# nnnagle/vq-vae

Measured on AMD Instinct MI355X. Metric: tiles/sec, higher is better.
Workload: dtype bf16

## Files before the change

include/frl_hip.h:

```cpp
#ifndef FRL_HIP_H
#define FRL_HIP_H

#include <stddef.h>
#include <stdint.h>

#ifdef __cplusplus
extern "C" {
#endif

typedef void* frl_stream_t;

enum { FRL_F32 = 0, FRL_BF16 = 1, FRL_F16 = 2  };
enum { FRL_ACT_NONE = 0, FRL_ACT_RELU = 1, FRL_ACT_SIGMOID = 2 };

int frl_version(void);
const char* frl_last_error(void);
int frl_device_arch(char* buf, int n);
int frl_kernel_timing_enable(int on);
int frl_kernel_timing_report(char* buf, int n);

size_t frl_pack_cache_table_bytes(void);
int frl_pack_cache_create(void* arena, size_t bytes);
int frl_pack_cache_destroy(int handle);
int frl_pack_cache_activate(int handle);
// ... 56 lines not shown
                     const float* b2, const float* stats, float* dw1, float* dg1, float* db1, float* dw2, float* dg2, float* db2,
                     int B, int HW, void* ws, size_t ws_bytes, frl_stream_t stream);

int frl_sobel_fwd(const void* x, void* g, int B, int H, int W, int C, int dtype, frl_stream_t stream);
int frl_sobel_bwd(const void* dg, void* dx, int B, int H, int W, int C, int dtype, frl_stream_t stream);
int frl_sobel_bwd_add(const void* dg, void* dx, const void* dx_add, int B, int H, int W, int C, int dtype, frl_stream_t stream);
int frl_edge_smooth_stencil_fwd(const void* x, const void* a_logit, const void* b_logit, void* smoothed, void* residual,
                                void* a_soft, void* b_soft, int B, int H, int W, int C, int R, int coarse_dilation,
                                int dtype, frl_stream_t stream);
int frl_edge_smooth_stencil_bwd(const void* d_smoothed, const void* x, const void* a_soft, const void* b_soft, void* dx,
                                void* da_logit, void* db_logit, const void* dx_add , int B, int H,
                                int W, int C, int R, int coarse_dilation, int dtype, frl_stream_t stream);
int frl_smooth_heads_supported(int C, int hidden, int rank, int dtype);
size_t frl_smooth_heads_workspace_bytes(int64_t npix);
int frl_smooth_heads_fwd(const void* x, const void* feat, const float* wa, const float* ba, const float* wb, const float* bb,
                         void* smoothed, void* residual, int B, int H, int W, int coarse_dilation, void* ws, size_t ws_bytes,
                         frl_stream_t stream);
size_t frl_smooth_heads_bwd_scratch_bytes(int64_t npix);
int frl_smooth_heads_force_gather(int on);
int frl_smooth_heads_bwd(const void* d_smoothed, const void* x, const void* feat, const float* wa, const float* ba, const float* wb,
                         const float* bb, const void* dx_add, void* dx, void* dfeat, float* dwa, float* dba, float* dwb, float* dbb,
                         void* scratch, size_t scratch_bytes, int B, int H, int W, int coarse_dilation, void* ws, size_t ws_bytes,
                         frl_stream_t stream);
int frl_smooth_heads_bwd_masked(const void* d_smoothed, const void* x, const void* feat, const float* wa, const float* ba, const float* wb,
                                const float* bb, const void* dx_add, void* dx, void* dfeat, float* dwa, float* dba, float* dwb, float* dbb,
                                void* scratch, size_t scratch_bytes, int B, int H, int W, int dil, int dfeat_relu, void* ws,
                                size_t ws_bytes, frl_stream_t stream);
int frl_film_fused_supported(int cond_dim, int hidden, int target_dim, int dtype);
size_t frl_film_fused_workspace_bytes(void);
int frl_film_fused_fwd(const void* z_type, const void* h, const float* w1g, const float* b1g, const float* w2g, const float* b2g,
                       const float* w1b, const float* b1b, const float* w2b, const float* b2b, void* z, void* gamma, void* beta, int B,
                       int T, int HW, void* ws, size_t ws_bytes, frl_stream_t stream);
int frl_film_fused_bwd(const void* z_type, const void* h, const void* dz, const float* w1g, const float* b1g, const float* w2g,
                       const float* b2g, const float* w1b, const float* b1b, const float* w2b, const float* b2b, void* dh, float* dw1g,
                       float* db1g, float* dw2g, float* db2g, float* dw1b, float* db1b, float* dw2b, float* db2b, int B, int T, int HW,
                       void* ws, size_t ws_bytes, frl_stream_t stream);
int frl_gate_blend_fwd(const void* smoothed, const void* residual, const void* gate_raw, float min_gate, void* out,
                       void* gate_out, int64_t n, int dtype, frl_stream_t stream);
int frl_gate_blend_bwd(const void* dout, const void* dgate_ext, const void* residual, const void* gate_raw, float min_gate,
                       void* d_residual, void* d_gate_raw, int64_t n, int dtype, frl_stream_t stream);
int frl_gate_blend_bwd_masked(const void* dout, const void* dgate_ext, const void* residual, const void* gate_raw, float min_gate,
                              void* d_residual, void* d_gate_raw, int64_t n, int dtype, int sigmoid_mask, frl_stream_t stream);

int frl_tcn_block_fwd(const void* x, const float* conv_w, const float* conv_b, const float* gn_w, const float* gn_b,
                      const float* gate_w, const float* gate_b, const float* proj_w, const float* proj_b, void* y,
                      int64_t npix, int HW, int T, int Cin, int Cout, int dilation, int G, float eps, int dtype, void* ws,
                      size_t ws_bytes, frl_stream_t stream);
size_t frl_tcn_block_bwd_workspace_bytes(int64_t npix, int Cout);
int frl_tcn_block_bwd(const void* x, const void* dy, const float* conv_w, const float* conv_b, const float* gn_w,
                      const float* gn_b, const float* gate_w, const float* gate_b, const float* proj_w,
                      const float* proj_b, void* dconv, void* dgpre, void* normed, void* dres, float* dgamma, float* dbeta,
                      int64_t npix, int HW, int T, int Cin, int Cout, int dilation, int G, float eps, int dtype, void* ws,
                      size_t ws_bytes, frl_stream_t stream);
int frl_tcn_block_bwd_data(const void* dconv, const void* dres, const float* conv_w, const float* proj_w, void* dx,
                           int64_t npix, int HW, int T, int Cin, int Cout, int dilation, int dtype, void* ws, size_t ws_bytes,
                           frl_stream_t stream);

int frl_tcn_block_bwd_fused_supported(int T, int Cin, int Cout, int G, int has_proj, int dtype);
size_t frl_tcn_block_bwd_fused_workspace_bytes(int64_t npix);
int frl_tcn_block_bwd_fused(const void* x, const void* dy, const float* conv_w, const float* conv_b, const float* gn_w,
                            const float* gn_b, const float* gate_w, const float* gate_b, void* dx, float* d_conv_w,
                            float* d_conv_b, float* d_gn_w, float* d_gn_b, float* d_gate_w, float* d_gate_b, int64_t npix,
                            int HW, int T, int dilation, int G, float eps, void* ws, size_t ws_bytes, frl_stream_t stream);

int frl_defer_begin(void);
int frl_defer_pending(void);
int frl_defer_destinations(void** out, int max);
int frl_defer_flush(frl_stream_t stream);
int frl_defer_abort(void);

int frl_tcn_hot_supported(int T, int Cin, int Cout, int G, int dilation, int has_proj, int dtype);
size_t frl_tcn_hot_fwd_workspace_bytes(void);
size_t frl_tcn_hot_bwd_workspace_bytes(int64_t npix);
int frl_tcn_hot_fwd(const void* x, const void* drop_mask, const float* conv_w, const float* conv_b, const float* gn_w, const float* gn_b,
                    const float* gate_w, const float* gate_b, void* y, int64_t npix, int HW, int dilation, float eps, void* ws,
                    size_t ws_bytes, frl_stream_t stream);
int frl_tcn_hot_bwd_nodx_supported(int64_t npix, int HW);
int frl_tcn_hot_bwd(const void* x, const void* drop_mask, const void* dy, const float* conv_w, const float* conv_b, const float* gn_w,
                    const float* gn_b, const float* gate_w, const float* gate_b, void* dx, float* d_conv_w, float* d_conv_b,
                    float* d_gn_w, float* d_gn_b, float* d_gate_w, float* d_gate_b, int64_t npix, int HW, int dilation,
                    float eps, void* ws, size_t ws_bytes, frl_stream_t stream);
size_t frl_tcn_chain_fwd_workspace_bytes(void);
int frl_tcn_chain_static_tiles(int on);
int frl_tcn_chain_fwd(const void* x, const float* const* conv_w, const float* const* conv_b, const float* const* gn_w,
                      const float* const* gn_b, const float* const* gate_w, const float* const* gate_b, const float* head_w,
                      const float* head_b, void* y1, void* y2, void* y3, void* h, int64_t npix, int HW, int Ch, float eps, void* ws,
                      size_t ws_bytes, frl_stream_t stream);
int frl_tcn_hot_bwd_head_supported(int64_t npix, int HW, int Ch);
size_t frl_tcn_hot_bwd_head_workspace_bytes(int64_t npix);
int frl_tcn_hot_bwd_head(const void* x, const void* dh, const float* head_w, int Ch, const float* conv_w, const float* conv_b,
                         const float* gn_w, const float* gn_b, const float* gate_w, const float* gate_b, void* dx, float* d_conv_w,
                         float* d_conv_b, float* d_gn_w, float* d_gn_b, float* d_gate_w, float* d_gate_b, int64_t npix, int HW,
                         int dilation, float eps, void* ws, size_t ws_bytes, frl_stream_t stream);
int frl_tcn_hot_force_generic_tiles(int on);
int frl_tcn_hot_bwd_variant(int v);
int frl_tcn_hot_bwd4_share(int variant, int share);

size_t frl_adamw_workspace_bytes(void);
int frl_adamw_clip_step(const void* desc_host, int ntensors, const void* chunks, const int* chunk_tensor, int nchunks, float max_norm,
                        float lr, double beta1, double beta2, float eps, int step, float* norm_out, const float* ok, int* counters,
                        const float* lr_dev, void* ws, size_t ws_bytes, frl_stream_t stream);
int frl_multi_tensor_scale_copy(const void* desc_host, int ntensors, const void* chunks, const int* chunk_tensor, int nchunks, float scale,
                                frl_stream_t stream);

int frl_film_modulate_fwd(const void* h, const void* gamma, const void* beta, void* out, int64_t B, int T, int64_t HW,
                          int C, int dtype, frl_stream_t stream);
int frl_film_modulate_bwd(const void* dout, const void* h, const void* gamma, void* dh, void* dgamma, void* dbeta,
                          int64_t B, int T, int64_t HW, int C, int dtype, frl_stream_t stream);
int frl_mean_time_fwd(const void* tile, void* out, int64_t B, int T, int64_t HWC, int dtype, frl_stream_t stream);
int frl_add(const void* a, const void* b, float scale_b, void* out, int64_t n, int dtype, frl_stream_t stream);

typedef struct FrlNormRec {
  float sub, div, mul, add, lo, hi;
  int flags;
  int pad;
} FrlNormRec;
int frl_normalize_tiles(const void* raw, int raw_dtype, const uint8_t* valid, const void* table, void* out, int out_dtype,
                        uint8_t* mask_out, int64_t rows, int F, frl_stream_t stream);
int frl_normalize_chunk_tiles(const void* chunk, int raw_dtype, int T, int CY, int CX, int F, const int32_t* desc, int ntiles,
                              int tile, const void* table, void* out, int out_dtype, uint8_t* mask_out, frl_stream_t stream);

int frl_host_parallel_copy(void* dst, const void* src, size_t nbytes, int nthreads);

size_t frl_mse_workspace_bytes(void);
int frl_mse_fwd(const void* pred, const void* target, const uint8_t* mask, int64_t P, int C, float* out, int dtype,
                void* ws, size_t ws_bytes, frl_stream_t stream);
int frl_mse_bwd(const void* pred, const void* target, const uint8_t* mask, const float* gscale, const float* stats,
                int64_t P, int C, void* dpred, int dtype, frl_stream_t stream);

int frl_decoder_mse_fused_supported(int Cz, int hidden, int F, int dtype);
size_t frl_decoder_mse_workspace_bytes(int64_t P, int Cz);
int frl_decoder_mse_fwd(const void* z, const float* w1, const float* b1, const float* w2, const float* b2, const void* target,
                        const uint8_t* mask, void* xhat, float* out, int64_t P, int Cz, void* ws, size_t ws_bytes,
                        frl_stream_t stream);
int frl_decoder_mse_bwd(const void* z, const float* w1, const float* b1, const float* w2, const float* b2, const void* target,
                        const uint8_t* mask, const float* gscale, const float* stats, void* dz, float* dw1, float* db1,
                        float* dw2, float* db2, int64_t P, int Cz, void* ws, size_t ws_bytes, frl_stream_t stream);
int frl_decoder_mse_bwd_subgroups(int on);

size_t frl_vq_workspace_bytes(int64_t N, int K, int d);
int frl_vq_assign_fwd(const void* z, const float* E, int64_t N, int K, int d, int32_t* idx_out, void* zq_out,
                      float* stats_out, int32_t* counts_out, int dtype, void* ws, size_t ws_bytes, frl_stream_t stream);
size_t frl_vq_prepared_bytes(int K, int d);
int frl_vq_stream_tiles(int nt);
int frl_vq_prepare(const float* E, int64_t N, int K, int d, int dtype, void* prep, size_t prep_bytes, frl_stream_t stream);
int frl_vq_assign_fwd_prepared(const void* z, const float* E, void* prep , int64_t N, int K, int d,
                               int32_t* idx_out, void* zq_out, float* stats_out, int32_t* counts_out, int dtype, void* ws,
                               size_t ws_bytes, frl_stream_t stream);
int frl_vq_bwd(const void* g_out, const void* z, const void* zq , const float* E, const int32_t* idx, const int32_t* counts,
               const float* gscale, float beta, int64_t N, int K, int d, void* g_z_out, float* g_E_out, float* sums_out,
               int dtype, void* ws, size_t ws_bytes, frl_stream_t stream);
int frl_vq_ema_update(const float* sums, const int32_t* counts, int K, int d, float decay, float eps, float* ema_count,
                      float* ema_sum, float* E, const float* ok, frl_stream_t stream);
int frl_vq_revive_dead_codes(float* E, const int64_t* window_counts, int64_t min_count, const void* z, int64_t N, int K, int d,
                             uint64_t seed, float* m, float* v, int32_t* revived, int dtype, frl_stream_t stream);

int frl_gather_locations_fwd(const void* feat, int64_t sC, int64_t sH, int64_t sW, int C, int H, int W, const int64_t* coords, int64_t N,
                             void* out, int dtype, frl_stream_t stream);
int frl_segment_sum_rows(const float* vals, const int64_t* order, const int64_t* keys_sorted, int64_t M, int D, float* out, int64_t out_stride,
                         int accumulate, frl_stream_t stream);
int frl_infonce_fwd(const float* emb, int D, const int64_t* pairs, const float* weights, const unsigned char* is_pos, int64_t T,
                    const int64_t* seg, int64_t nseg, float temperature, int similarity, float* sims, float* logits, float* loss_a, float* coef,
                    float* loss, frl_stream_t stream);
int frl_infonce_pair_grads(const float* emb, int D, const int64_t* pairs, const float* sims, const float* coef, const float* gscale, int64_t T,
                           int64_t nseg, float temperature, int similarity, float* ga, float* gb, frl_stream_t stream);

// ... 12 lines not shown
```

vq-vae_amd/csrc/tcn_hot.hip:

```cpp
#include "tcn_hot_common.hpp"

#ifdef TH_STAMPS
__device__ unsigned long long* th_dbg;
#endif
#define TH_PITCH 72

struct Tile2 { frag8 f[2]; };

__device__ __forceinline__ float th_elem(const Tile2& t, int j) { return (float)t.f[j >> 3][j & 7]; }

__device__ __forceinline__ Tile2 th_pack(const float (&v)[16]) {
  Tile2 o;
#pragma unroll
  for (int j = 0; j < 16; ++j) o.f[j >> 3][j & 7] = (bf16)v[j];
  return o;
}

template <int DIL>
__device__ __forceinline__ void th_conv(f32x4 (&acc)[TH_T][4], const Tile2 (&x)[TH_T], const frag8* __restrict__ wl, int lane) {
#pragma unroll
  for (int k = 0; k < 3; ++k)
#pragma unroll
    for (int m = 0; m < 4; ++m)
#pragma unroll
// ... 196 lines not shown
template <bool KEEP>
__global__ __launch_bounds__(512, 2) void tcn_chain_fwd_kernel(const bf16* __restrict__ X, ThChainArgs a, int64_t npix, int HW, int Ch, float eps, int dyn) {
  extern __shared__ __attribute__((aligned(16))) char smem[];
  frag8* wl = reinterpret_cast<frag8*>(smem);
  frag8* wlh = wl + 3 * THC_IMG;
  float* tab = reinterpret_cast<float*>(wlh + 2 * 64);
  const int tid = threadIdx.x, lane = tid & 63, wave = tid >> 6;
  const int px = lane & 15, kc = lane >> 4;
#pragma unroll
  for (int b = 0; b < 3; ++b) copy_frags_lds<bf16>(wl + b * THC_IMG, a.pk[b], THC_IMG, tid, 512);
  copy_frags_lds<bf16>(wlh, a.pkh, 2 * 64, tid, 512);
  for (int i = tid; i < 3 * 256 + 16; i += 512) {
    float v;
    if (i < 768) {
      const int b = i >> 8, w = (i >> 6) & 3, c = i & 63;
      v = w == 0 ? a.bc[b][c] : w == 1 ? a.gw[b][c] : w == 2 ? a.gb[b][c] : -1.44269504088896f * a.bg[b][c];
    } else {
      v = (i - 768) < Ch ? a.bh[i - 768] : 0.f;
    }
    tab[i] = v;
  }
  int* tctr = reinterpret_cast<int*>(tab + 3 * 256 + 16);
  if (tid == 0) *tctr = 8;
  __syncthreads();
  const int64_t ntile = (npix + 15) >> 4;
  const int64_t tstep = (int64_t)gridDim.x * 8;
  auto tile_of = [&](int i) -> int64_t { return (int64_t)blockIdx.x * 8 + (i & 7) + (int64_t)(i >> 3) * tstep; };
  auto rows = [&](int64_t tile, bool& valid) -> int64_t {
    int64_t pidx = tile * 16 + px;
    valid = pidx < npix;
    if (!valid) pidx = npix - 1;
    const int64_t b = pidx / HW, hw = pidx % HW;
    return (b * TH_T * HW + hw) * 64 + 16 * kc;
  };
  Tile2 x[TH_T];
  {
    bool v;
    const int64_t t0 = tile_of(wave);
    const int64_t r0 = rows(t0 < ntile ? t0 : 0, v);
#pragma unroll
    for (int t = 0; t < TH_T; ++t) x[t] = th_load(X + r0 + (int64_t)t * HW * 64);
  }
  int icur = wave;
  for (int64_t tile = tile_of(wave); tile < ntile;) {
    bool valid, vn;
    int inext = icur + 8;
    if (dyn && lane == 0) inext = __hip_atomic_fetch_add(tctr, 1, __ATOMIC_RELAXED, __HIP_MEMORY_SCOPE_WORKGROUP);
    const int64_t r0 = rows(tile, valid);
    int lw = lane, z0 = 0;
    asm volatile("" : "+v"(lw), "+s"(z0));
    const float* tb_ = tab + z0;
    th_block_regs<1>(x, wl, wl + 24 * 64, tb_, lw, kc, eps);
    if (KEEP && valid) {
#pragma unroll
      for (int t = 0; t < TH_T; ++t) th_store(a.y[0] + r0 + (int64_t)t * HW * 64, x[t]);
    }
    __builtin_amdgcn_sched_barrier(0);
    th_block_regs<2>(x, wl + THC_IMG, wl + THC_IMG + 24 * 64, tb_ + 256, lw, kc, eps);
    if (KEEP && valid) {
#pragma unroll
      for (int t = 0; t < TH_T; ++t) th_store(a.y[1] + r0 + (int64_t)t * HW * 64, x[t]);
    }
    __builtin_amdgcn_sched_barrier(0);
    th_block_regs<4>(x, wl + 2 * THC_IMG, wl + 2 * THC_IMG + 24 * 64, tb_ + 512, lw, kc, eps);
    __builtin_amdgcn_sched_barrier(0);
    const f32x4 hb4 = *reinterpret_cast<const f32x4*>(tb_ + 768 + 4 * kc);
    const int64_t hrow = (r0 - 16 * kc) / 64 * Ch + 4 * kc;
#pragma unroll
    for (int t = 0; t < TH_T; ++t) {
      if (KEEP && valid) th_store(a.y[2] + r0 + (int64_t)t * HW * 64, x[t]);
      f32x4 ha = mfma16(wlh[lw], x[t].f[0], hb4);
      ha = mfma16(wlh[64 + lw], x[t].f[1], ha);
      if (valid && 4 * kc < Ch)
        *reinterpret_cast<bf16x4*>(a.h + hrow + (int64_t)t * HW * Ch) = bf16x4{(bf16)ha[0], (bf16)ha[1], (bf16)ha[2], (bf16)ha[3]};
    }
    {
      icur = __builtin_amdgcn_readfirstlane(inext);
      const int64_t tnext = tile_of(icur);
      const int64_t rn = rows(tnext < ntile ? tnext : tile, vn);
#pragma unroll
      for (int t = 0; t < TH_T; ++t) x[t] = th_load(X + rn + (int64_t)t * HW * 64);
      tile = tnext;
    }
  }
}

__device__ __forceinline__ frag8 th_tr(const bf16* tile, int pix0, int ch0, int r16) {
  const bf16* a0 = tile + (pix0 + (r16 >> 2)) * TH_PITCH + ch0 + 4 * (r16 & 3);
  bf16x4 lo = __builtin_amdgcn_ds_read_tr16_b64_v4bf16((bf16x4 __attribute__((address_space(3)))*)(a0));
  bf16x4 hi = __builtin_amdgcn_ds_read_tr16_b64_v4bf16((bf16x4 __attribute__((address_space(3)))*)(a0 + 4 * TH_PITCH));
  return frag8{lo[0], lo[1], lo[2], lo[3], hi[0], hi[1], hi[2], hi[3]};
}
__device__ __forceinline__ void th_put(bf16* tile, int prow, int kc, const Tile2& t) {
  frag8* p = reinterpret_cast<frag8*>(tile + prow * TH_PITCH + 16 * kc);
  p[0] = t.f[0];
  p[1] = t.f[1];
}

#define TH_TILE (64 * TH_PITCH)

__device__ __forceinline__ Tile2 th_get(const bf16* tile, int prow, int kc) {
  const frag8* p = reinterpret_cast<const frag8*>(tile + prow * TH_PITCH + 16 * kc);
  Tile2 t;
  t.f[0] = p[0];
  t.f[1] = p[1];
  return t;
}

template <int DIL, bool MASK>
__global__ __launch_bounds__(512, 2) void tcn_hot_bwd2_kernel(const bf16* __restrict__ X, const bf16* __restrict__ M, const bf16* __restrict__ DY,
                                                              const frag8* __restrict__ Wpk, const float* __restrict__ bc,
                                                              const float* __restrict__ gn_w, const float* __restrict__ gn_b,
                                                              const float* __restrict__ bg, bf16* DX, float* __restrict__ slab,
                                                              int64_t npix, int HW, float eps) {
  extern __shared__ __attribute__((aligned(16))) char smem[];
  frag8* wl_conv = reinterpret_cast<frag8*>(smem);
  frag8* wl_gate = wl_conv + 24 * 64;
  frag8* wl_gateT = wl_gate + 8 * 64;
  frag8* wl_convT = wl_gateT + 8 * 64;
  float* tab = reinterpret_cast<float*>(wl_convT + 24 * 64);
  float* gacc_lds = tab + 4 * 64;
  bf16* bufA = reinterpret_cast<bf16*>(gacc_lds + 4 * 2 * 64);
  bf16* bufB = bufA + TH_T * TH_TILE;
  const int tid = threadIdx.x, lane = tid & 63, wave = tid >> 6;
  const int q = wave & 3, h = wave >> 2;
  const int px = lane & 15, kc = lane >> 4, r16 = px;
  const int prow = q * 16 + px;
  const int co = 16 * kc + 8 * h;
#ifdef TH_STAMPS
  __shared__ unsigned long long th_ts[8][12];
  if (tid < 96) (&th_ts[0][0])[tid] = 0ull;
  unsigned long long t_prev = 0;
#define TH_ST2(i) do { const unsigned long long t_now = __builtin_amdgcn_s_memtime(); if (lane == 0) th_ts[wave][i] += t_now - t_prev; t_prev = t_now; } while (0)
#else
#define TH_ST2(i) do { } while (0)
#endif

  copy_frags_lds<bf16>(wl_conv, Wpk, 64 * 64, tid, 512);
  if (tid < 64) {
    tab[tid] = bc[tid];
    tab[64 + tid] = gn_w[tid];
    tab[128 + tid] = gn_b[tid];
    tab[192 + tid] = -1.44269504088896f * bg[tid];
  }
  __syncthreads();
  float gw[8], gb[8];
#pragma unroll
  for (int e = 0; e < 8; ++e) { gw[e] = tab[64 + co + e]; gb[e] = tab[128 + co + e]; }
  const float* tnbg = tab + 192 + co;
  const f32x4* tcb = reinterpret_cast<const f32x4*>(tab + co);
  const frag8* wc_own = wl_conv + (2 * h) * 2 * 64 + lane;
  const frag8* wg_own = wl_gate + (2 * h) * 2 * 64 + lane;
  const frag8* wgT_own = wl_gateT + (2 * h) * 2 * 64 + lane;
  const frag8* wcT_own = wl_convT + (2 * h) * 2 * 64 + lane;

  f32x4 accC[3][2], accG[2], accCb = {0.f, 0.f, 0.f, 0.f}, accGb = {0.f, 0.f, 0.f, 0.f};
#pragma unroll
  for (int k = 0; k < 3; ++k)
#pragma unroll
    for (int i = 0; i < 2; ++i) accC[k][i] = f32x4{0.f, 0.f, 0.f, 0.f};
#pragma unroll
  for (int i = 0; i < 2; ++i) accG[i] = f32x4{0.f, 0.f, 0.f, 0.f};
  float dgam[8], dbet[8];
#pragma unroll
  for (int e = 0; e < 8; ++e) { dgam[e] = 0.f; dbet[e] = 0.f; }
  const frag8 ones = (r16 == 0) ? frag8{(bf16)1.f, (bf16)1.f, (bf16)1.f, (bf16)1.f, (bf16)1.f, (bf16)1.f, (bf16)1.f, (bf16)1.f}
// ... 295 lines not shown
  return (unsigned)g;
}
static constexpr size_t TH_FWD_LDS = (size_t)32 * 64 * sizeof(frag8) + 4 * 64 * sizeof(float);
static constexpr size_t TH_BWD_LDS = TH_PACK_BYTES + (size_t)(4 * 64 + 4 * 2 * 64) * sizeof(float) + (size_t)2 * TH_T * TH_TILE * sizeof(bf16);

template <int DIL>
static int th_launch_fwd(const void* x, const void* mask, const frag8* pk, const float* bc, const float* gw, const float* gb, const float* bg,
                         void* y, int64_t npix, int HW, float eps, hipStream_t st) {
  if (mask != nullptr) {
    FRL_LAUNCH((tcn_hot_fwd_kernel<DIL, true>), dim3(th_fwd_grid(npix)), dim3(256), TH_FWD_LDS, st, (const bf16*)x, (const bf16*)mask, pk, bc, gw,
               gb, bg, (bf16*)y, npix, HW, eps);
  } else {
    FRL_LAUNCH((tcn_hot_fwd_kernel<DIL, false>), dim3(th_fwd_grid(npix)), dim3(256), TH_FWD_LDS, st, (const bf16*)x, (const bf16*)nullptr, pk, bc,
               gw, gb, bg, (bf16*)y, npix, HW, eps);
  }
  return 0;
}
template <int DIL>
static int th_launch_bwd(const void* x, const void* mask, const void* dy, const frag8* pk, const float* bc, const float* gw, const float* gb,
                         const float* bg, void* dx, float* slab, unsigned grid, int64_t npix, int HW, float eps, hipStream_t st) {
  if (mask != nullptr) {
    auto kern = tcn_hot_bwd2_kernel<DIL, true>;
    FRL_HIP(hipFuncSetAttribute((const void*)kern, hipFuncAttributeMaxDynamicSharedMemorySize, (int)TH_BWD_LDS));
    FRL_LAUNCH_AS("tcn_hot_bwd2_kernel", kern, dim3(grid), dim3(512), TH_BWD_LDS, st, (const bf16*)x, (const bf16*)mask, (const bf16*)dy, pk, bc, gw, gb, bg, (bf16*)dx,
               slab, npix, HW, eps);
  } else {
    auto kern = tcn_hot_bwd2_kernel<DIL, false>;
    FRL_HIP(hipFuncSetAttribute((const void*)kern, hipFuncAttributeMaxDynamicSharedMemorySize, (int)TH_BWD_LDS));
    FRL_LAUNCH_AS("tcn_hot_bwd2_kernel", kern, dim3(grid), dim3(512), TH_BWD_LDS, st, (const bf16*)x, (const bf16*)nullptr, (const bf16*)dy, pk, bc, gw, gb, bg, (bf16*)dx,
               slab, npix, HW, eps);
  }
  return 0;
}

static int g_th_force_bwd2 = 0;

static const frag8* th_packed(const float* conv_w, const float* gate_w, frag8* ws_pk, hipStream_t stream) {
  FrlPackJob jobs[8];
  const size_t blk = (size_t)4 * 2 * 64 * sizeof(frag8);
  for (int k = 0; k < 3; ++k) jobs[k] = frl_pack_job_pw(conv_w + k, k * blk, FRL_BF16, 2, 64, 64, 4, 64 * 3, 3);
  jobs[3] = frl_pack_job_pw(gate_w, 3 * blk, FRL_BF16, 2, 64, 64, 4, 64, 1);
  jobs[4] = frl_pack_job_pw(gate_w, 4 * blk, FRL_BF16, 2, 64, 64, 4, 1, 64);
  for (int k = 0; k < 3; ++k) jobs[5 + k] = frl_pack_job_pw(conv_w + k, (5 + k) * blk, FRL_BF16, 2, 64, 64, 4, 3, 64 * 3);
  bool hit = false;
  frag8* pk = ws_pk;
  if (void* img = frl_pack_cached(jobs, 8, TH_PACK_BYTES, &hit)) pk = (frag8*)img;
  if (!hit) FRL_LAUNCH(tcn_hot_pack_kernel, dim3(32), dim3(256), 0, stream, pk, conv_w, gate_w);
  return pk;
}

extern "C" {

int frl_tcn_hot_force_generic_tiles(int on) { const int was = g_th_force_bwd2; g_th_force_bwd2 = on; return was; }
static int g_th_bwd_variant = 4;
int frl_tcn_hot_bwd_variant(int v) { const int was = g_th_bwd_variant; if (v == 3 || v == 4) g_th_bwd_variant = v; return was; }

int frl_tcn_hot_supported(int T, int Cin, int Cout, int G, int dilation, int has_proj, int dtype) {
  return dtype == FRL_BF16 && Cin == 64 && Cout == 64 && T == TH_T && G == 8 && !has_proj && (dilation == 1 || dilation == 2 || dilation == 4);
}

int frl_tcn_hot_bwd_nodx_supported(int64_t npix, int HW) { return (th_bwd3_supported(npix, HW) && !g_th_force_bwd2) ? 1 : 0; }

size_t frl_tcn_hot_fwd_workspace_bytes(void) { return TH_PACK_BYTES; }
size_t frl_tcn_hot_bwd_workspace_bytes(int64_t npix) { return (size_t)th_bwd_grid(npix) * TH_SLAB * sizeof(float) + 256 + TH_PACK_BYTES; }

int frl_tcn_hot_fwd(const void* x, const void* drop_mask, const float* conv_w, const float* conv_b, const float* gn_w, const float* gn_b, const float* gate_w,
                    const float* gate_b, void* y, int64_t npix, int HW, int dilation, float eps, void* ws, size_t ws_bytes,
                    hipStream_t stream) {
  if (npix <= 0 || HW <= 0) return frl_fail(-2, "tcn_hot_fwd: empty input");
  if (ws == nullptr || ws_bytes < TH_PACK_BYTES) return frl_fail(-4, "tcn_hot_fwd: workspace too small");
  const frag8* pk = th_packed(conv_w, gate_w, (frag8*)ws, stream);
  int rc = -2;
  if (dilation == 1) rc = th_launch_fwd<1>(x, drop_mask, pk, conv_b, gn_w, gn_b, gate_b, y, npix, HW, eps, stream);
  else if (dilation == 2) rc = th_launch_fwd<2>(x, drop_mask, pk, conv_b, gn_w, gn_b, gate_b, y, npix, HW, eps, stream);
  else if (dilation == 4) rc = th_launch_fwd<4>(x, drop_mask, pk, conv_b, gn_w, gn_b, gate_b, y, npix, HW, eps, stream);
  else return frl_fail(-2, "tcn_hot_fwd: dilation must be 1, 2 or 4");
  if (rc) return rc;
  return frl_check_launch("tcn_hot_fwd");
}

size_t frl_tcn_chain_fwd_workspace_bytes(void) { return 3 * TH_PACK_BYTES + 4096; }
static int g_thc_static = 0;
int frl_tcn_chain_static_tiles(int on) { const int was = g_thc_static; g_thc_static = on ? 1 : 0; return was; }
int frl_tcn_chain_fwd(const void* x, const float* const* conv_w, const float* const* conv_b, const float* const* gn_w, const float* const* gn_b,
                      const float* const* gate_w, const float* const* gate_b, const float* head_w, const float* head_b, void* y1, void* y2, void* y3,
                      void* h, int64_t npix, int HW, int Ch, float eps, void* ws, size_t ws_bytes, hipStream_t stream) {
  if (npix <= 0 || HW <= 0) return frl_fail(-2, "tcn_chain_fwd: empty input");
  if (Ch < 4 || Ch > 16 || (Ch & 3)) return frl_fail(-2, "tcn_chain_fwd: head width must be 4, 8, 12 or 16");
  if (ws == nullptr || ws_bytes < frl_tcn_chain_fwd_workspace_bytes()) return frl_fail(-4, "tcn_chain_fwd: workspace too small");
  const int n_keep = (y1 != nullptr) + (y2 != nullptr) + (y3 != nullptr);
  if (n_keep != 0 && n_keep != 3) return frl_fail(-2, "tcn_chain_fwd: y1, y2, y3 must be all set (training) or all NULL (inference)");
  if (h == nullptr) return frl_fail(-1, "tcn_chain_fwd: h is NULL");
  const bool keep = n_keep == 3;
  ThChainArgs a;
  char* w = (char*)ws;
  for (int b = 0; b < 3; ++b) {
    a.pk[b] = th_packed(conv_w[b], gate_w[b], reinterpret_cast<frag8*>(w + b * TH_PACK_BYTES), stream);
    a.bc[b] = conv_b[b]; a.gw[b] = gn_w[b]; a.gb[b] = gn_b[b]; a.bg[b] = gate_b[b];
  }
  {
    FrlPackJob job = frl_pack_job_pw(head_w, 0, FRL_BF16, 2, Ch, 64, 1, 64, 1);
    bool hit = false;
    frag8* pk = reinterpret_cast<frag8*>(w + 3 * TH_PACK_BYTES);
    if (void* img = frl_pack_cached(&job, 1, (size_t)2 * 64 * sizeof(frag8), &hit)) pk = (frag8*)img;
    if (!hit) FRL_LAUNCH((pack_weights_kernel<bf16, 2>), dim3(1), dim3(128), 0, stream, pk, head_w, Ch, 64, 1, (int64_t)64, (int64_t)1);
    a.pkh = pk;
  }
  a.bh = head_b;
  a.y[0] = (bf16*)y1; a.y[1] = (bf16*)y2; a.y[2] = (bf16*)y3; a.h = (bf16*)h;
  int64_t g = ((npix + 15) / 16 + 7) / 8;
  if (g > 256) g = 256;
  const size_t lds = (size_t)(3 * THC_IMG + 2 * 64) * sizeof(frag8) + (3 * 256 + 16) * sizeof(float) + 16;
  if (keep) {
    FRL_HIP(hipFuncSetAttribute((const void*)tcn_chain_fwd_kernel<true>, hipFuncAttributeMaxDynamicSharedMemorySize, (int)lds));
    FRL_LAUNCH_AS("tcn_chain_fwd_kernel", tcn_chain_fwd_kernel<true>, dim3((unsigned)g), dim3(512), lds, stream, (const bf16*)x, a, npix, HW, Ch, eps, g_thc_static ? 0 : 1);
  } else {
    FRL_HIP(hipFuncSetAttribute((const void*)tcn_chain_fwd_kernel<false>, hipFuncAttributeMaxDynamicSharedMemorySize, (int)lds));
    FRL_LAUNCH_AS("tcn_chain_fwd_kernel<false>", tcn_chain_fwd_kernel<false>, dim3((unsigned)g), dim3(512), lds, stream, (const bf16*)x, a, npix, HW, Ch, eps, g_thc_static ? 0 : 1);
  }
  return frl_check_launch("tcn_chain_fwd");
}

int frl_tcn_hot_bwd(const void* x, const void* drop_mask, const void* dy, const float* conv_w, const float* conv_b, const float* gn_w, const float* gn_b,
                    const float* gate_w, const float* gate_b, void* dx, float* d_conv_w, float* d_conv_b, float* d_gn_w, float* d_gn_b,
                    float* d_gate_w, float* d_gate_b, int64_t npix, int HW, int dilation, float eps, void* ws, size_t ws_bytes,
                    hipStream_t stream) {
  if (npix <= 0 || HW <= 0) return frl_fail(-2, "tcn_hot_bwd: empty input");
  if (npix >= (int64_t)1 << 31) return frl_fail(-2, "tcn_hot_bwd: more than 2^31 pixels per launch");
  if (ws == nullptr || ws_bytes < frl_tcn_hot_bwd_workspace_bytes(npix)) return frl_fail(-4, "tcn_hot_bwd: workspace too small");
  const unsigned grid = th_bwd_grid(npix);
  float* slab = (float*)ws;
  const frag8* pk = th_packed(conv_w, gate_w,
                              reinterpret_cast<frag8*>(reinterpret_cast<char*>(ws) + (((size_t)grid * TH_SLAB * sizeof(float) + 255) / 256) * 256), stream);
  int rc = -2;
  if (dx == nullptr && !(drop_mask == nullptr && th_bwd3_supported(npix, HW) && !g_th_force_bwd2))
    return frl_fail(-2, "tcn_hot_bwd: dx may be NULL (input without gradient) only on the tcn_hot_bwd3 route (no mask, HW % 64 == 0)");
  if (drop_mask == nullptr && th_bwd3_supported(npix, HW) && !g_th_force_bwd2)
    rc = (g_th_bwd_variant == 4 && th_bwd4_supported(npix, HW))
             ? th_bwd4_launch(dilation, x, dy, pk, conv_b, gn_w, gn_b, gate_b, dx, slab, grid, npix, HW, eps, stream)
             : th_bwd3_launch(dilation, x, dy, pk, conv_b, gn_w, gn_b, gate_b, dx, slab, grid, npix, HW, eps, stream);
  else if (dilation == 1) rc = th_launch_bwd<1>(x, drop_mask, dy, pk, conv_b, gn_w, gn_b, gate_b, dx, slab, grid, npix, HW, eps, stream);
  else if (dilation == 2) rc = th_launch_bwd<2>(x, drop_mask, dy, pk, conv_b, gn_w, gn_b, gate_b, dx, slab, grid, npix, HW, eps, stream);
  else if (dilation == 4) rc = th_launch_bwd<4>(x, drop_mask, dy, pk, conv_b, gn_w, gn_b, gate_b, dx, slab, grid, npix, HW, eps, stream);
  else return frl_fail(-2, "tcn_hot_bwd: dilation must be 1, 2 or 4");
  if (rc) return rc;
  launch_slab_reduce_deferrable<float, ThEpi>((const float*)slab, (int)grid, (int64_t)TH_SLAB, ThEpi{d_conv_w, d_gate_w, d_conv_b, d_gate_b, d_gn_w, d_gn_b},
                                   stream);
  return frl_check_launch("tcn_hot_bwd");
}

int frl_tcn_hot_bwd_head_supported(int64_t npix, int HW, int Ch) {
  return (th_bwd4_supported(npix, HW) && !g_th_force_bwd2 && g_th_bwd_variant == 4 && Ch >= 4 && Ch <= 16 && (Ch & 3) == 0) ? 1 : 0;
}
size_t frl_tcn_hot_bwd_head_workspace_bytes(int64_t npix) { return frl_tcn_hot_bwd_workspace_bytes(npix) + 4096; }
int frl_tcn_hot_bwd_head(const void* x, const void* dh, const float* head_w, int Ch, const float* conv_w, const float* conv_b, const float* gn_w,
                         const float* gn_b, const float* gate_w, const float* gate_b, void* dx, float* d_conv_w, float* d_conv_b, float* d_gn_w,
                         float* d_gn_b, float* d_gate_w, float* d_gate_b, int64_t npix, int HW, int dilation, float eps, void* ws, size_t ws_bytes,
                         hipStream_t stream) {
  if (npix <= 0 || HW <= 0) return frl_fail(-2, "tcn_hot_bwd_head: empty input");
  if (!frl_tcn_hot_bwd_head_supported(npix, HW, Ch)) return frl_fail(-2, "tcn_hot_bwd_head: unsupported shape (HW % 64, head width 4..16 in fours)");
  if (ws == nullptr || ws_bytes < frl_tcn_hot_bwd_head_workspace_bytes(npix)) return frl_fail(-4, "tcn_hot_bwd_head: workspace too small");
  const unsigned grid = th_bwd_grid(npix);
  float* slab = (float*)ws;
  char* wpk = reinterpret_cast<char*>(ws) + (((size_t)grid * TH_SLAB * sizeof(float) + 255) / 256) * 256;
  const frag8* pk = th_packed(conv_w, gate_w, reinterpret_cast<frag8*>(wpk), stream);
  const frag8* whp;
  {
    FrlPackJob job = frl_pack_job_pw(head_w, 0, FRL_BF16, 1, 64, Ch, 4, 1, 64);
    bool hit = false;
    frag8* img = reinterpret_cast<frag8*>(wpk + TH_PACK_BYTES);
    if (void* c = frl_pack_cached(&job, 1, (size_t)4 * 64 * sizeof(frag8), &hit)) img = (frag8*)c;
    if (!hit) FRL_LAUNCH((pack_weights_kernel<bf16, 1>), dim3(1), dim3(256), 0, stream, img, head_w, 64, Ch, 4, (int64_t)1, (int64_t)64);
    whp = img;
  }
  const int rc = th_bwd4_launch(dilation, x, dh, pk, conv_b, gn_w, gn_b, gate_b, dx, slab, grid, npix, HW, eps, stream, whp, Ch);
  if (rc) return rc;
  launch_slab_reduce_deferrable<float, ThEpi>((const float*)slab, (int)grid, (int64_t)TH_SLAB, ThEpi{d_conv_w, d_gate_w, d_conv_b, d_gate_b, d_gn_w, d_gn_b},
                                   stream);
  return frl_check_launch("tcn_hot_bwd_head");
}

}
```

vq-vae_amd/frl_hip/_lib.py:

```python
from __future__ import annotations

import ctypes
import os
from ctypes import c_char_p, c_float, c_int, c_int64, c_size_t, c_void_p

_HERE = os.path.dirname(os.path.abspath(__file__))
LIB_PATH = os.path.join(_HERE, "libfrlhip_%s.so" % os.environ["FRL_HIP_LIB_TAG"] if os.environ.get("FRL_HIP_LIB_TAG") else "libfrlhip.so")

F32, BF16, F16 = 0, 1, 2
ACT_NONE, ACT_RELU, ACT_SIGMOID = 0, 1, 2

_lib = None


class FrlHipError(RuntimeError):
    pass


P, I, L, F, S, D = c_void_p, c_int, c_int64, c_float, c_size_t, ctypes.c_double
SIGNATURES = {
    "frl_version": (c_int, []),
    "frl_last_error": (c_char_p, []),
    "frl_device_arch": (c_int, [c_char_p, I]),
    "frl_kernel_timing_enable": (c_int, [I]),
# ... 17 lines not shown
    "frl_vq_workspace_bytes": (S, [L, I, I]),
    "frl_vq_assign_fwd": (c_int, [P, P, L, I, I, P, P, P, P, I, P, S, P]),
    "frl_vq_prepared_bytes": (S, [I, I]),
    "frl_vq_prepare": (c_int, [P, L, I, I, I, P, S, P]),
    "frl_vq_stream_tiles": (c_int, [I]),
    "frl_vq_assign_fwd_prepared": (c_int, [P, P, P, L, I, I, P, P, P, P, I, P, S, P]),
    "frl_vq_bwd": (c_int, [P, P, P, P, P, P, P, F, L, I, I, P, P, P, I, P, S, P]),
    "frl_vq_ema_update": (c_int, [P, P, I, I, F, F, P, P, P, P, P]),
    "frl_vq_revive_dead_codes": (c_int, [P, P, L, P, L, I, I, ctypes.c_uint64, P, P, P, I, P]),
    "frl_groupnorm_fwd": (c_int, [P, P, P, P, P, P, I, I, I, I, F, I, I, P]),
    "frl_groupnorm_bwd_workspace_bytes": (S, [I, I, I]),
    "frl_groupnorm_bwd": (c_int, [P, P, P, P, P, P, P, P, P, I, I, I, I, I, I, P, S, P]),
    "frl_scalar_combine": (c_int, [P, P, I, P, P, P]),
    "frl_scalar_fanout": (c_int, [P, P, I, P, P]),
    "frl_scalar_combine_dev": (c_int, [P, P, P, I, P, P, P]),
    "frl_scalar_combine_aux": (c_int, [P, P, P, P, I, P, P, P, P]),
    "frl_scalar_fanout_dev": (c_int, [P, P, P, I, P, P]),
    "frl_encoder2_supported": (c_int, [I, I, I, I, I, I, I]),
    "frl_encoder2_workspace_bytes": (S, [I]),
    "frl_encoder2_fwd": (c_int, [P, P, P, P, P, P, P, P, P, I, I, F, P, S, P]),
    "frl_encoder2_bwd": (c_int, [P, P, P, P, P, P, P, P, P, P, P, P, P, P, P, I, I, P, S, P]),
    "frl_decoder_mse_fused_supported": (c_int, [I, I, I, I]),
    "frl_decoder_mse_workspace_bytes": (S, [L, I]),
    "frl_decoder_mse_fwd": (c_int, [P, P, P, P, P, P, P, P, P, L, I, P, S, P]),
    "frl_decoder_mse_bwd": (c_int, [P, P, P, P, P, P, P, P, P, P, P, P, P, P, L, I, P, S, P]),
    "frl_mse_workspace_bytes": (S, []),
    "frl_mse_fwd": (c_int, [P, P, P, L, I, P, I, P, S, P]),
    "frl_mse_bwd": (c_int, [P, P, P, P, P, L, I, P, I, P]),
    "frl_film_modulate_fwd": (c_int, [P, P, P, P, L, I, L, I, I, P]),
    "frl_film_modulate_bwd": (c_int, [P, P, P, P, P, P, L, I, L, I, I, P]),
    "frl_film_fused_supported": (c_int, [I, I, I, I]),
    "frl_film_fused_workspace_bytes": (S, []),
    "frl_film_fused_fwd": (c_int, [P] * 13 + [I, I, I, P, S, P]),
    "frl_film_fused_bwd": (c_int, [P] * 20 + [I, I, I, P, S, P]),
    "frl_gate_blend_fwd": (c_int, [P, P, P, F, P, P, L, I, P]),
    "frl_gate_blend_bwd": (c_int, [P, P, P, P, F, P, P, L, I, P]),
    "frl_mean_time_fwd": (c_int, [P, P, L, I, L, I, P]),
    "frl_add": (c_int, [P, P, F, P, L, I, P]),
    "frl_normalize_tiles": (c_int, [P, I, P, P, P, I, P, L, I, P]),
    "frl_gather_locations_fwd": (c_int, [P, L, L, L, I, I, I, P, L, P, I, P]),
    "frl_segment_sum_rows": (c_int, [P, P, P, L, I, P, L, I, P]),
    "frl_infonce_fwd": (c_int, [P, I, P, P, P, L, P, L, F, I, P, P, P, P, P, P]),
    "frl_infonce_pair_grads": (c_int, [P, I, P, P, P, P, L, L, F, I, P, P, P]),
    "frl_mutual_knn_max_points": (S, [I]),
    "frl_mutual_knn": (c_int, [P, I, I, P, P, F, I, P, P, P]),
    "frl_host_parallel_copy": (c_int, [P, P, S, I]),
    "frl_normalize_chunk_tiles": (c_int, [P, I, I, I, I, I, P, I, I, P, P, I, P, P]),
    "frl_conv3x3_fwd": (c_int, [P, P, P, P, I, I, I, I, I, I, I, P, S, P]),
    "frl_conv3x3_fwd_gate_blend": (c_int, [P, P, P, P, P, P, P, I, I, I, I, I, I, P, S, P]),
    "frl_conv3x3_bwd_data": (c_int, [P, P, I, P, P, I, I, I, I, I, I, P, S, P]),
    "frl_conv3x3_bwd_data_fused": (c_int, [P, P, I, P, P, P, P, P, I, I, I, I, I, I, P, S, P]),
    "frl_conv3x3_bwd_weight_workspace_bytes": (S, [I, I, I, I, I]),
    "frl_conv3x3_bwd_weight": (c_int, [P, P, I, P, P, P, I, I, I, I, I, I, P, S, I, P]),
    "frl_sobel_fwd": (c_int, [P, P, I, I, I, I, I, P]),
    "frl_sobel_bwd": (c_int, [P, P, I, I, I, I, I, P]),
    "frl_sobel_bwd_add": (c_int, [P, P, P, I, I, I, I, I, P]),
    "frl_edge_smooth_stencil_fwd": (c_int, [P, P, P, P, P, P, P, I, I, I, I, I, I, I, P]),
    "frl_edge_smooth_stencil_bwd": (c_int, [P, P, P, P, P, P, P, P, I, I, I, I, I, I, I, P]),
    "frl_smooth_heads_supported": (c_int, [I, I, I, I]),
    "frl_smooth_heads_workspace_bytes": (S, [L]),
    "frl_smooth_heads_bwd_scratch_bytes": (S, [L]),
    "frl_smooth_heads_force_gather": (c_int, [I]),
    "frl_smooth_heads_fwd": (c_int, [P, P, P, P, P, P, P, P, I, I, I, I, P, S, P]),
    "frl_smooth_heads_bwd": (c_int, [P, P, P, P, P, P, P, P, P, P, P, P, P, P, P, S, I, I, I, I, P, S, P]),
    "frl_tcn_block_fwd": (c_int, [P, P, P, P, P, P, P, P, P, P, L, I, I, I, I, I, I, F, I, P, S, P]),
    "frl_tcn_block_bwd_data": (c_int, [P, P, P, P, P, L, I, I, I, I, I, I, P, S, P]),
    "frl_tcn_block_bwd_workspace_bytes": (S, [L, I]),
    "frl_tcn_block_bwd_fused_supported": (c_int, [I, I, I, I, I, I]),
    "frl_tcn_block_bwd_fused_workspace_bytes": (S, [L]),
    "frl_tcn_block_bwd_fused": (c_int, [P, P, P, P, P, P, P, P, P, P, P, P, P, P, P, L, I, I, I, I, F, P, S, P]),
    "frl_adamw_workspace_bytes": (S, []),
    "frl_adamw_clip_step": (c_int, [P, I, P, P, I, F, F, D, D, F, I, P, P, P, P, P, S, P]),
    "frl_multi_tensor_scale_copy": (c_int, [P, I, P, P, I, F, P]),
    "frl_tcn_hot_supported": (c_int, [I, I, I, I, I, I, I]),
    "frl_tcn_hot_fwd_workspace_bytes": (S, []),
    "frl_tcn_hot_bwd_workspace_bytes": (S, [L]),
    "frl_tcn_hot_fwd": (c_int, [P, P, P, P, P, P, P, P, P, L, I, I, F, P, S, P]),
    "frl_tcn_hot_bwd": (c_int, [P, P, P, P, P, P, P, P, P, P, P, P, P, P, P, P, L, I, I, F, P, S, P]),
    "frl_tcn_hot_force_generic_tiles": (c_int, [I]),
    "frl_tcn_hot_bwd_variant": (c_int, [I]),
    "frl_decoder_mse_bwd_subgroups": (c_int, [I]),
    "frl_tcn_hot_bwd4_share": (c_int, [I, I]),
    "frl_tcn_chain_static_tiles": (c_int, [I]),
    "frl_conv3x3_bwd_data_outmask": (c_int, [P, P, I, P, P, P, I, I, I, I, I, I, I, P, S, P]),
    "frl_gate_blend_bwd_masked": (c_int, [P, P, P, P, F, P, P, L, I, I, P]),
    "frl_smooth_heads_bwd_masked": (c_int, [P, P, P, P, P, P, P, P, P, P, P, P, P, P, P, S, I, I, I, I, I, P, S, P]),
    "frl_tcn_hot_bwd_head_supported": (c_int, [L, I, I]),
    "frl_tcn_hot_bwd_head_workspace_bytes": (S, [L]),
    "frl_tcn_hot_bwd_head": (c_int, [P, P, P, I, P, P, P, P, P, P, P, P, P, P, P, P, P, L, I, I, F, P, S, P]),
    "frl_defer_begin": (c_int, []),
    "frl_defer_pending": (c_int, []),
    "frl_defer_destinations": (c_int, [P, I]),
    "frl_defer_flush": (c_int, [P]),
    "frl_defer_abort": (c_int, []),
    "frl_tcn_hot_bwd_nodx_supported": (c_int, [L, I]),
    "frl_tcn_chain_fwd_workspace_bytes": (S, []),
    "frl_tcn_chain_fwd": (c_int, [P] * 13 + [L, I, I, F, P, S, P]),
    "frl_tcn_block_bwd": (c_int, [P, P, P, P, P, P, P, P, P, P, P, P, P, P, P, P, L, I, I, I, I, I, I, F, I, P, S, P]),
    "frl_decode_codes": (c_int, [P, P, P, L, I, I, I, P, P]),
}


def load():
    global _lib
    if _lib is not None:
        return _lib
    if not os.path.exists(LIB_PATH):
        raise FrlHipError(
            f"{LIB_PATH} not found: build it with `python vq-vae_amd/build.py` "
            "(hipcc --offload-arch=gfx950). There is no CPU fallback.")
    import torch
    lib = ctypes.CDLL(LIB_PATH)
    for name, (res, args) in SIGNATURES.items():
        fn = getattr(lib, name)
        fn.restype = res
        fn.argtypes = args
    _lib = lib
    return lib


def check(rc: int, what: str = "") -> None:
    if rc != 0:
        msg = load().frl_last_error()
        raise FrlHipError(f"{what} failed with code {rc}: {msg.decode() if msg else ''}")
```

Before: 100,700.

## Add 1024-thread chain forward kernel splitting each tile across wave pairs

Adds a new TCN chain forward kernel in which each 16-pixel tile is processed by two waves. Each wave computes half of the output channels, and the halves are exchanged through LDS using a lightweight per-pair atomic barrier. The grid uses 1024-thread blocks instead of 512, and this variant becomes the default when indices fit in 32 bits. The aim is to raise parallelism and latency hiding by halving per-wave MFMA work and register pressure per tile, at the cost of intra-pair spin synchronisation, extra LDS traffic and a duplicated group-norm reduction.

```diff
diff --git a/include/frl_hip.h b/include/frl_hip.h
--- a/include/frl_hip.h
+++ b/include/frl_hip.h
@@ -162,6 +162,7 @@
                     float eps, void* ws, size_t ws_bytes, frl_stream_t stream);
 size_t frl_tcn_chain_fwd_workspace_bytes(void);
 int frl_tcn_chain_static_tiles(int on);
+int frl_tcn_chain_variant(int v);
 int frl_tcn_chain_fwd(const void* x, const float* const* conv_w, const float* const* conv_b, const float* const* gn_w,
                       const float* const* gn_b, const float* const* gate_w, const float* const* gate_b, const float* head_w,
                       const float* head_b, void* y1, void* y2, void* y3, void* h, int64_t npix, int HW, int Ch, float eps, void* ws,
diff --git a/vq-vae_amd/csrc/tcn_hot.hip b/vq-vae_amd/csrc/tcn_hot.hip
--- a/vq-vae_amd/csrc/tcn_hot.hip
+++ b/vq-vae_amd/csrc/tcn_hot.hip
@@ -302,6 +302,216 @@
       for (int t = 0; t < TH_T; ++t) x[t] = th_load(X + rn + (int64_t)t * HW * 64);
       tile = tnext;
     }
+  }
+}
+
+__device__ __forceinline__ void thc4_sync(unsigned* bar, unsigned& gen, int lane) {
+  gen += 2u;
+  if (lane == 0) __hip_atomic_fetch_add(bar, 1u, __ATOMIC_RELAXED, __HIP_MEMORY_SCOPE_WORKGROUP);
+  for (;;) {
+    const unsigned seen = (unsigned)__builtin_amdgcn_readfirstlane((int)__hip_atomic_load(bar, __ATOMIC_RELAXED, __HIP_MEMORY_SCOPE_WORKGROUP));
+    if ((int)(seen - gen) >= 0) break;
+    __builtin_amdgcn_s_sleep(1);
+  }
+}
+#define THC4_SYNC() do { asm volatile("s_waitcnt lgkmcnt(0)" ::: "memory"); thc4_sync(bar, bgen, lw); asm volatile("" ::: "memory"); } while (0)
+
+struct Thc4Tail {
+  const frag8* wlh;
+  const float* hb;
+  bf16* h;
+  int Ch;
+  int64_t hstride;
+  bool hstore;
+  const bf16* X;
+  unsigned xnext;
+};
+
+template <int DIL, bool LAST, bool KEEP>
+__device__ __forceinline__ void thc4_block(Tile2 (&x)[TH_T], const frag8* __restrict__ wl_conv, const frag8* __restrict__ wl_gate,
+                                           const float* __restrict__ tab, int lw, int kc, int h, float eps, frag8* ex, unsigned* bar,
+                                           unsigned& bgen, bf16* __restrict__ yo, unsigned ro, bool valid, int64_t tstride, const Thc4Tail& tl) {
+  const int co = 16 * kc + 8 * h;
+  const f32x4* tcb = reinterpret_cast<const f32x4*>(tab + co);
+  const float* tgw0 = tab + 64 + co;
+  const float* tgb0 = tab + 128 + co;
+  const float* tnbg0 = tab + 192 + co;
+  const frag8* wc = wl_conv + (2 * h) * 2 * 64 + lw;
+  const frag8* wg = wl_gate + (2 * h) * 2 * 64 + lw;
+  f32x4 acc[TH_T][2];
+#pragma unroll
+  for (int mm = 0; mm < 2; ++mm) {
+    const f32x4 cb = tcb[mm];
+#pragma unroll
+    for (int t = 0; t < TH_T; ++t) acc[t][mm] = cb;
+  }
+#pragma unroll
+  for (int k = 0; k < 3; ++k)
+#pragma unroll
+    for (int mm = 0; mm < 2; ++mm)
+#pragma unroll
+      for (int s = 0; s < 2; ++s) {
+        const frag8 wf = wc[((k * 4 + mm) * 2 + s) * 64];
+#pragma unroll
+        for (int t = 0; t < TH_T; ++t)
+          if (th_valid<DIL>(t, k)) acc[t][mm] = mfma16(wf, x[t + (k - 1) * DIL].f[s], acc[t][mm]);
+      }
+  __builtin_amdgcn_sched_barrier(0);
+  float nm, rstd;
+  {
+    f32x4 s = f32x4{0.f, 0.f, 0.f, 0.f};
+#pragma unroll
+    for (int t = 0; t < TH_T; ++t)
+#pragma unroll
+      for (int m = 0; m < 2; ++m)
+#pragma unroll
+        for (int r = 0; r < 4; ++r) s[r] += acc[t][m][r];
+    const float mu = ((s[0] + s[1]) + (s[2] + s[3])) * (1.f / 40.f);
+    f32x4 q = f32x4{0.f, 0.f, 0.f, 0.f};
+#pragma unroll
+    for (int t = 0; t < TH_T; ++t)
+#pragma unroll
+      for (int m = 0; m < 2; ++m)
+#pragma unroll
+        for (int r = 0; r < 4; ++r) { const float d = acc[t][m][r] - mu; q[r] = fmaf(d, d, q[r]); }
+    rstd = 1.f / sqrtf(((q[0] + q[1]) + (q[2] + q[3])) * (1.f / 40.f) + eps);
+    nm = -mu * rstd;
+  }
+  frag8* exA = ex + lw;
+  frag8* exB = ex + 2 * 64 + lw;
+#pragma unroll
+  for (int t = 0; t < TH_T; ++t) {
+    __builtin_amdgcn_sched_barrier(0);
+    int zt = 0;
+    asm volatile("" : "+s"(zt));
+    const float* tgw = tgw0 + zt;
+    const float* tgb = tgb0 + zt;
+    const float* tnbg = tnbg0 + zt;
+    float n[8];
+#pragma unroll
+    for (int e = 0; e < 8; ++e) n[e] = fmaf(fmaf(acc[t][e >> 2][e & 3], rstd, nm), tgw[e], tgb[e]);
+    exA[h * 64] = th_pack8(n);
+    THC4_SYNC();
+    const frag8 n0 = exA[0], n1 = exA[64];
+    f32x4 gacc[2];
+#pragma unroll
+    for (int mm = 0; mm < 2; ++mm) {
+      gacc[mm] = mfma16(wg[(mm * 2 + 0) * 64], n0, f32x4{0.f, 0.f, 0.f, 0.f});
+      gacc[mm] = mfma16(wg[(mm * 2 + 1) * 64], n1, gacc[mm]);
+    }
+    const frag8 xr = h ? x[t].f[1] : x[t].f[0];
+    float y[8];
+#pragma unroll
+    for (int e = 0; e < 8; ++e) {
+      const float g = __builtin_amdgcn_rcpf(1.f + __builtin_amdgcn_exp2f(fmaf(gacc[e >> 2][e & 3], -1.44269504088896f, tnbg[e])));
+      const float o = fmaxf(n[e], 0.f);
+      const float res = (float)xr[e];
+      y[e] = fmaf(g, o - res, res);
+    }
+    const frag8 yb = th_pack8(y);
+    exB[h * 64] = yb;
+    if (KEEP && valid) *reinterpret_cast<frag8*>(yo + t * tstride + (size_t)ro) = yb;
+    THC4_SYNC();
+    if constexpr (!LAST) {
+      x[t].f[0] = exB[0];
+      x[t].f[1] = exB[64];
+    } else {
+      if ((t & 1) == h) {
+        f32x4 ha = mfma16(tl.wlh[lw], exB[0], *reinterpret_cast<const f32x4*>(tl.hb));
+        ha = mfma16(tl.wlh[64 + lw], exB[64], ha);
+        if (tl.hstore) *reinterpret_cast<bf16x4*>(tl.h + t * tl.hstride + (size_t)((ro >> 6) * (unsigned)tl.Ch + 4u * (unsigned)kc)) = bf16x4{(bf16)ha[0], (bf16)ha[1], (bf16)ha[2], (bf16)ha[3]};
+      }
+      x[t] = th_load(tl.X + t * tstride + (size_t)tl.xnext);
+    }
+  }
+}
+
+#define THC4_CTL 32
+#define THC4_EX (2 * 2 * 64)
+template <bool KEEP>
+__global__ __launch_bounds__(1024) void tcn_chain_fwd_kernel_w4(const bf16* __restrict__ X, ThChainArgs a, int64_t npix, int HW, int Ch, float eps, int dyn) {
+  extern __shared__ __attribute__((aligned(16))) char smem[];
+  frag8* wl = reinterpret_cast<frag8*>(smem);
+  frag8* wlh = wl + 3 * THC_IMG;
+  float* tab = reinterpret_cast<float*>(wlh + 2 * 64);
+  int* ctl = reinterpret_cast<int*>(tab + 3 * 256 + 16);
+  const int tid = threadIdx.x;
+  const int wave = __builtin_amdgcn_readfirstlane(tid >> 6);
+  const int p = wave >> 1, h = wave & 1;
+  frag8* ex = reinterpret_cast<frag8*>(ctl + THC4_CTL) + p * THC4_EX;
+  unsigned* bar = reinterpret_cast<unsigned*>(ctl + 8 + p);
+  int* pnext = ctl + 16 + p;
+#pragma unroll
+  for (int b = 0; b < 3; ++b) copy_frags_lds<bf16>(wl + b * THC_IMG, a.pk[b], THC_IMG, tid, 1024);
+  copy_frags_lds<bf16>(wlh, a.pkh, 2 * 64, tid, 1024);
+  for (int i = tid; i < 3 * 256 + 16; i += 1024) {
+    float v;
+    if (i < 768) {
+      const int b = i >> 8, w = (i >> 6) & 3, c = i & 63;
+      v = w == 0 ? a.bc[b][c] : w == 1 ? a.gw[b][c] : w == 2 ? a.gb[b][c] : -1.44269504088896f * a.bg[b][c];
+    } else {
+      v = (i - 768) < Ch ? a.bh[i - 768] : 0.f;
+    }
+    tab[i] = v;
+  }
+  if (tid < THC4_CTL) ctl[tid] = tid == 0 ? 8 : 0;
+  __syncthreads();
+  unsigned bgen = 0;
+  const int64_t ntile = (npix + 15) >> 4;
+  const int64_t tstep = (int64_t)gridDim.x * 8;
+  const int64_t tstride = (int64_t)HW * 64;
+  auto tile_of = [&](int i) -> int64_t { return (int64_t)blockIdx.x * 8 + (i & 7) + (int64_t)(i >> 3) * tstep; };
+  auto lane_id = [&]() -> int {
+    int l;
+    asm volatile("v_mbcnt_lo_u32_b32 %0, -1, 0\n\tv_mbcnt_hi_u32_b32 %0, -1, %0" : "=v"(l));
+    return l;
+  };
+  auto rows = [&](int64_t tile, int lw, bool& valid) -> unsigned {
+    const int px = lw & 15, kc = lw >> 4;
+    int hw_ = HW;
+    asm volatile("" : "+s"(hw_));
+    const unsigned HWu = (unsigned)hw_;
+    unsigned pidx = (unsigned)tile * 16u + (unsigned)px;
+    valid = pidx < (unsigned)npix;
+    if (!valid) pidx = (unsigned)npix - 1u;
+    const unsigned b = pidx / HWu, hw = pidx - b * HWu;
+    return (b * (TH_T * HWu) + hw) * 64u + 16u * (unsigned)kc;
+  };
+  Tile2 x[TH_T];
+  {
+    bool v;
+    const int64_t t0 = tile_of(p);
+    const unsigned r0 = rows(t0 < ntile ? t0 : 0, lane_id(), v);
+#pragma unroll
+    for (int t = 0; t < TH_T; ++t) x[t] = th_load(X + t * tstride + (size_t)r0);
+  }
+  int icur = p;
+  Thc4Tail tl;
+  tl.wlh = wlh;
+  tl.h = a.h;
+  tl.Ch = Ch;
+  tl.X = X;
+  tl.hstride = (int64_t)HW * Ch;
+  for (int64_t tile = tile_of(p); tile < ntile;) {
+    bool valid, vn;
+    const int lw = lane_id(), kc = lw >> 4;
+    if (dyn && h == 0 && lw == 0) *pnext = __hip_atomic_fetch_add(ctl, 1, __ATOMIC_RELAXED, __HIP_MEMORY_SCOPE_WORKGROUP);
+    const unsigned r0 = rows(tile, lw, valid);
+    int z0 = 0;
+    asm volatile("" : "+s"(z0));
+    const float* tb_ = tab + z0;
+    thc4_block<1, false, KEEP>(x, wl, wl + 24 * 64, tb_, lw, kc, h, eps, ex, bar, bgen, a.y[0] + 8 * h, r0, valid, tstride, tl);
+    __builtin_amdgcn_sched_barrier(0);
+    icur = dyn ? __builtin_amdgcn_readfirstlane(*pnext) : icur + 8;
+    const int64_t tnext = tile_of(icur);
+    thc4_block<2, false, KEEP>(x, wl + THC_IMG, wl + THC_IMG + 24 * 64, tb_ + 256, lw, kc, h, eps, ex, bar, bgen, a.y[1] + 8 * h, r0, valid, tstride, tl);
+    __builtin_amdgcn_sched_barrier(0);
+    tl.hb = tb_ + 768 + 4 * kc;
+    tl.hstore = valid && 4 * kc < Ch;
+    tl.xnext = rows(tnext < ntile ? tnext : tile, lw, vn);
+    thc4_block<4, true, KEEP>(x, wl + 2 * THC_IMG, wl + 2 * THC_IMG + 24 * 64, tb_ + 512, lw, kc, h, eps, ex, bar, bgen, a.y[2] + 8 * h, r0, valid, tstride, tl);
+    __builtin_amdgcn_sched_barrier(0);
+    tile = tnext;
   }
 }
 
@@ -763,6 +973,8 @@
 size_t frl_tcn_chain_fwd_workspace_bytes(void) { return 3 * TH_PACK_BYTES + 4096; }
 static int g_thc_static = 0;
 int frl_tcn_chain_static_tiles(int on) { const int was = g_thc_static; g_thc_static = on ? 1 : 0; return was; }
+static int g_thc_variant = 4;
+int frl_tcn_chain_variant(int v) { const int was = g_thc_variant; if (v == 2 || v == 4) g_thc_variant = v; return was; }
 int frl_tcn_chain_fwd(const void* x, const float* const* conv_w, const float* const* conv_b, const float* const* gn_w, const float* const* gn_b,
                       const float* const* gate_w, const float* const* gate_b, const float* head_w, const float* head_b, void* y1, void* y2, void* y3,
                       void* h, int64_t npix, int HW, int Ch, float eps, void* ws, size_t ws_bytes, hipStream_t stream) {
@@ -791,13 +1003,26 @@
   a.y[0] = (bf16*)y1; a.y[1] = (bf16*)y2; a.y[2] = (bf16*)y3; a.h = (bf16*)h;
   int64_t g = ((npix + 15) / 16 + 7) / 8;
   if (g > 256) g = 256;
+  const int dyn = g_thc_static ? 0 : 1;
+  if (g_thc_variant == 4 && npix * TH_T * 64 < ((int64_t)1 << 31)) {
+    const size_t lds4 = (size_t)(3 * THC_IMG + 2 * 64) * sizeof(frag8) + (3 * 256 + 16) * sizeof(float) + THC4_CTL * sizeof(int) +
+                        (size_t)8 * THC4_EX * sizeof(frag8);
+    if (keep) {
+      FRL_HIP(hipFuncSetAttribute((const void*)tcn_chain_fwd_kernel_w4<true>, hipFuncAttributeMaxDynamicSharedMemorySize, (int)lds4));
+      FRL_LAUNCH_AS("tcn_chain_fwd_kernel_w4", tcn_chain_fwd_kernel_w4<true>, dim3((unsigned)g), dim3(1024), lds4, stream, (const bf16*)x, a, npix, HW, Ch, eps, dyn);
+    } else {
+      FRL_HIP(hipFuncSetAttribute((const void*)tcn_chain_fwd_kernel_w4<false>, hipFuncAttributeMaxDynamicSharedMemorySize, (int)lds4));
+      FRL_LAUNCH_AS("tcn_chain_fwd_kernel_w4<false>", tcn_chain_fwd_kernel_w4<false>, dim3((unsigned)g), dim3(1024), lds4, stream, (const bf16*)x, a, npix, HW, Ch, eps, dyn);
+    }
+    return frl_check_launch("tcn_chain_fwd");
+  }
   const size_t lds = (size_t)(3 * THC_IMG + 2 * 64) * sizeof(frag8) + (3 * 256 + 16) * sizeof(float) + 16;
   if (keep) {
     FRL_HIP(hipFuncSetAttribute((const void*)tcn_chain_fwd_kernel<true>, hipFuncAttributeMaxDynamicSharedMemorySize, (int)lds));
-    FRL_LAUNCH_AS("tcn_chain_fwd_kernel", tcn_chain_fwd_kernel<true>, dim3((unsigned)g), dim3(512), lds, stream, (const bf16*)x, a, npix, HW, Ch, eps, g_thc_static ? 0 : 1);
+    FRL_LAUNCH_AS("tcn_chain_fwd_kernel", tcn_chain_fwd_kernel<true>, dim3((unsigned)g), dim3(512), lds, stream, (const bf16*)x, a, npix, HW, Ch, eps, dyn);
   } else {
     FRL_HIP(hipFuncSetAttribute((const void*)tcn_chain_fwd_kernel<false>, hipFuncAttributeMaxDynamicSharedMemorySize, (int)lds));
-    FRL_LAUNCH_AS("tcn_chain_fwd_kernel<false>", tcn_chain_fwd_kernel<false>, dim3((unsigned)g), dim3(512), lds, stream, (const bf16*)x, a, npix, HW, Ch, eps, g_thc_static ? 0 : 1);
+    FRL_LAUNCH_AS("tcn_chain_fwd_kernel<false>", tcn_chain_fwd_kernel<false>, dim3((unsigned)g), dim3(512), lds, stream, (const bf16*)x, a, npix, HW, Ch, eps, dyn);
   }
   return frl_check_launch("tcn_chain_fwd");
 }
diff --git a/vq-vae_amd/frl_hip/_lib.py b/vq-vae_amd/frl_hip/_lib.py
--- a/vq-vae_amd/frl_hip/_lib.py
+++ b/vq-vae_amd/frl_hip/_lib.py
@@ -123,6 +123,7 @@
     "frl_decoder_mse_bwd_subgroups": (c_int, [I]),
     "frl_tcn_hot_bwd4_share": (c_int, [I, I]),
     "frl_tcn_chain_static_tiles": (c_int, [I]),
+    "frl_tcn_chain_variant": (c_int, [I]),
     "frl_conv3x3_bwd_data_outmask": (c_int, [P, P, I, P, P, P, I, I, I, I, I, I, I, P, S, P]),
     "frl_gate_blend_bwd_masked": (c_int, [P, P, P, P, F, P, P, L, I, I, P]),
     "frl_smooth_heads_bwd_masked": (c_int, [P, P, P, P, P, P, P, P, P, P, P, P, P, P, P, S, I, I, I, I, I, P, S, P]),
```

Result: faster. 101,700, median of 6 (+1.1%).
